# gongweibao/FleetX

Hardware: AMD Instinct MI355X
Metric: tokens/sec (whole node) GPT-3 6.7B hybrid-parallel at 1/2/4/8 MI355X (higher is better)
Workload: dtype bf16; 1 GPU; model=gpt3-6.7B, global_batch=8, seq_len=1024, parallelism=dp1, micro_batch=8, hip_graph=True, grad_reduce_dtype=float32, recompute=False

## Files before the change

### csrc/kernels/norm_eltwise.hip

```cpp
#include "fx_api.h"
#include "fx_common.h"

namespace {

struct DropCfg {
  uint32_t klo, khi, thr;
  float scale;
  int enabled;
  const uint64_t* salt;
};

__device__ __forceinline__ DropCfg resolve_drop(DropCfg d) {
  if (d.enabled && d.salt != nullptr) {
    const uint64_t k = salt_key(((uint64_t)d.khi << 32) | d.klo, *d.salt);
    d.klo = (uint32_t)k;
    d.khi = (uint32_t)(k >> 32);
  }
  return d;
}

__device__ __forceinline__ float drop_apply(float v, uint64_t idx, const DropCfg& d) {
  if (!d.enabled) return v;
  uint32_t h = elem_rand_pair(idx, d.klo, d.khi);
  uint32_t r = (idx & 1) ? (h >> 16) : (h & 0xffffu);
// ... 83 lines not shown
  for (int i = 0; i < VPT; ++i) {
    if (MASK && (i * 64 + lane) * 8 >= h) continue;
#pragma unroll
    for (int j = 0; j < 8; ++j) {
      float d = v[i][j] - mean;
      var += d * d;
    }
  }
  const float rstd = rsqrtf(wave_sum(var) / h + eps);
#pragma unroll
  for (int i = 0; i < VPT; ++i) {
    const int c = (i * 64 + lane) * 8;
    if (MASK && c >= h) continue;
    float g[8], b[8], o[8];
    load8<T>(gamma + c, g);
    load8<T>(beta + c, b);
#pragma unroll
    for (int j = 0; j < 8; ++j) o[j] = (v[i][j] - mean) * rstd * g[j] + b[j];
    store8<T>(y + base + c, o);
  }
  if (lane == 0) {
    mean_out[row] = mean;
    rstd_out[row] = rstd;
  }
}

template <typename T>
__global__ __launch_bounds__(256) void add_ln_fwd_generic(
    const uint16_t* __restrict__ x, const uint16_t* __restrict__ bias,
    const uint16_t* __restrict__ residual, const uint16_t* __restrict__ gamma,
    const uint16_t* __restrict__ beta, uint16_t* __restrict__ s_out,
    uint16_t* __restrict__ y, float* __restrict__ mean_out, float* __restrict__ rstd_out,
    int rows, int h, float eps, DropCfg drop_) {
  const DropCfg drop = resolve_drop(drop_);
  const int lane = threadIdx.x & 63;
  const int row = blockIdx.x * 4 + (threadIdx.x >> 6);
  if (row >= rows) return;
  const size_t base = (size_t)row * h;
  const int nv = h / 8;
  auto value = [&](int c, float* v) {
    load8<T>(x + base + c, v);
    if (bias) {
      float b[8];
      load8<T>(bias + c, b);
      for (int j = 0; j < 8; ++j) v[j] += b[j];
    }
    if (drop.enabled)
      drop_apply8(v, base + c, drop);
    if (residual) {
      float r[8];
      load8<T>(residual + base + c, r);
      for (int j = 0; j < 8; ++j) v[j] += r[j];
    }
  };
  float sum = 0.f;
  for (int vi = lane; vi < nv; vi += 64) {
    float v[8];
    value(vi * 8, v);
    if (s_out) {
      store8<T>(s_out + base + vi * 8, v);
      for (int j = 0; j < 8; ++j) v[j] = round_to<T>(v[j]);
    }
    for (int j = 0; j < 8; ++j) sum += v[j];
  }
  const float mean = wave_sum(sum) / h;
  float var = 0.f;
  for (int vi = lane; vi < nv; vi += 64) {
    float v[8];
    if (s_out) load8<T>(s_out + base + vi * 8, v); else value(vi * 8, v);
    for (int j = 0; j < 8; ++j) { float d = v[j] - mean; var += d * d; }
  }
  const float rstd = rsqrtf(wave_sum(var) / h + eps);
  for (int vi = lane; vi < nv; vi += 64) {
    float v[8], g[8], b[8], o[8];
    if (s_out) load8<T>(s_out + base + vi * 8, v); else value(vi * 8, v);
    load8<T>(gamma + vi * 8, g);
    load8<T>(beta + vi * 8, b);
    for (int j = 0; j < 8; ++j) o[j] = (v[j] - mean) * rstd * g[j] + b[j];
    store8<T>(y + base + vi * 8, o);
  }
  if (lane == 0) { mean_out[row] = mean; rstd_out[row] = rstd; }
}

template <typename T, int VPT, bool MASK = false>
__global__ __launch_bounds__(256) void ln_bwd_row_kernel(
    const uint16_t* __restrict__ dy, const uint16_t* __restrict__ s,
    const float* __restrict__ mean_in, const float* __restrict__ rstd_in,
    const uint16_t* __restrict__ gamma, const uint16_t* __restrict__ ds_in,
    uint16_t* __restrict__ ds_out, uint16_t* __restrict__ dx_out, int rows, int h,
    DropCfg drop_) {
  const DropCfg drop = resolve_drop(drop_);
  const int lane = threadIdx.x & 63;
  const int row = blockIdx.x * 4 + (threadIdx.x >> 6);
  if (row >= rows) return;
  const size_t base = (size_t)row * h;
  const float mean = mean_in[row], rstd = rstd_in[row];
  float xh[VPT][8], gdy[VPT][8];
  float s1 = 0.f, s2 = 0.f;
#pragma unroll
  for (int i = 0; i < VPT; ++i) {
    const int c = (i * 64 + lane) * 8;
    if (MASK && c >= h) {
#pragma unroll
      for (int j = 0; j < 8; ++j) xh[i][j] = gdy[i][j] = 0.f;
      continue;
    }
    float a[8], g[8], d[8];
    load8<T>(s + base + c, a);
    load8<T>(gamma + c, g);
    load8<T>(dy + base + c, d);
#pragma unroll
    for (int j = 0; j < 8; ++j) {
      xh[i][j] = (a[j] - mean) * rstd;
      gdy[i][j] = d[j] * g[j];
      s1 += gdy[i][j];
      s2 += gdy[i][j] * xh[i][j];
    }
  }
  uint4 dr[VPT];
  if (ds_in) {
#pragma unroll
    for (int i = 0; i < VPT; ++i) {
      const int c = (i * 64 + lane) * 8;
      dr[i] = make_uint4(0, 0, 0, 0);
      if (!MASK || c < h) dr[i] = *reinterpret_cast<const uint4*>(ds_in + base + c);
    }
  }
  const float m1 = wave_sum(s1) / h, m2 = wave_sum(s2) / h;
#pragma unroll
  for (int i = 0; i < VPT; ++i) {
    const int c = (i * 64 + lane) * 8;
    if (MASK && c >= h) continue;
    float o[8];
#pragma unroll
    for (int j = 0; j < 8; ++j) o[j] = rstd * (gdy[i][j] - m1 - xh[i][j] * m2);
    if (ds_in) {
      float r[8];
      unpack8<T>(dr[i], r);
#pragma unroll
      for (int j = 0; j < 8; ++j) o[j] += r[j];
    }
    store8<T>(ds_out + base + c, o);
    if (drop.enabled) {
      drop_apply8(o, base + c, drop);
      store8<T>(dx_out + base + c, o);
    } else if (dx_out != ds_out) {
      store8<T>(dx_out + base + c, o);
    }
  }
}

template <typename T>
__global__ __launch_bounds__(256) void ln_bwd_row_generic(
    const uint16_t* __restrict__ dy, const uint16_t* __restrict__ s,
    const float* __restrict__ mean_in, const float* __restrict__ rstd_in,
    const uint16_t* __restrict__ gamma, const uint16_t* __restrict__ ds_in,
    uint16_t* __restrict__ ds_out, uint16_t* __restrict__ dx_out, int rows, int h,
    DropCfg drop_) {
  const DropCfg drop = resolve_drop(drop_);
  const int lane = threadIdx.x & 63;
  const int row = blockIdx.x * 4 + (threadIdx.x >> 6);
  if (row >= rows) return;
  const size_t base = (size_t)row * h;
  const float mean = mean_in[row], rstd = rstd_in[row];
  const int nv = h / 8;
  float s1 = 0.f, s2 = 0.f;
  for (int vi = lane; vi < nv; vi += 64) {
    float a[8], g[8], d[8];
    load8<T>(s + base + vi * 8, a);
    load8<T>(gamma + vi * 8, g);
    load8<T>(dy + base + vi * 8, d);
    for (int j = 0; j < 8; ++j) {
      float xh = (a[j] - mean) * rstd, gd = d[j] * g[j];
      s1 += gd;
      s2 += gd * xh;
    }
  }
  const float m1 = wave_sum(s1) / h, m2 = wave_sum(s2) / h;
  for (int vi = lane; vi < nv; vi += 64) {
    const int c = vi * 8;
    float a[8], g[8], d[8], o[8];
    load8<T>(s + base + c, a);
    load8<T>(gamma + c, g);
    load8<T>(dy + base + c, d);
    for (int j = 0; j < 8; ++j) o[j] = rstd * (d[j] * g[j] - m1 - (a[j] - mean) * rstd * m2);
    if (ds_in) {
      float r[8];
      load8<T>(ds_in + base + c, r);
      for (int j = 0; j < 8; ++j) o[j] += r[j];
    }
    store8<T>(ds_out + base + c, o);
    if (drop.enabled) {
      drop_apply8(o, base + c, drop);
      store8<T>(dx_out + base + c, o);
    } else if (dx_out != ds_out) {
      store8<T>(dx_out + base + c, o);
    }
  }
}

template <typename T, int VPT, int WPR, bool MASK, bool DB>
__global__ __launch_bounds__(256, 2) void ln_bwd_cols_kernel(
    const uint16_t* __restrict__ dy, const uint16_t* __restrict__ s,
    const float* __restrict__ mean_in, const float* __restrict__ rstd_in,
    const uint16_t* __restrict__ gamma, const uint16_t* __restrict__ ds_in,
    uint16_t* __restrict__ ds_out, uint16_t* __restrict__ dx_out, int rows, int h,
    int rows_per_group, float* __restrict__ part, DropCfg drop_) {
  constexpr int NG = 4 / WPR;
  __shared__ float red[4 * 512 * VPT];
  __shared__ float xs[2][4][2];
  const DropCfg drop = resolve_drop(drop_);
  const int lane = threadIdx.x & 63, w = threadIdx.x >> 6;
  const int grp = w / WPR, half = w % WPR;
  const int hw = h / WPR, cbase = half * hw;
  const int r0 = min(rows, (blockIdx.x * NG + grp) * rows_per_group);
  const int r1 = min(rows, r0 + rows_per_group);
  uint4 gp[VPT];
  float ag[VPT][8], ab[VPT][8], ax[DB ? VPT : 1][8];
#pragma unroll
  for (int i = 0; i < VPT; ++i) {
    const int c = (i * 64 + lane) * 8;
    gp[i] = (!MASK || c < hw) ? *reinterpret_cast<const uint4*>(gamma + cbase + c)
                              : make_uint4(0, 0, 0, 0);
#pragma unroll
    for (int j = 0; j < 8; ++j) {
      ag[i][j] = ab[i][j] = 0.f;
      if (DB) ax[i][j] = 0.f;
    }
  }
  for (int k = 0; k < rows_per_group; ++k) {
    const int r = r0 + k;
    const bool live = r < r1;
    if (WPR == 1 && !live) break;
    const size_t base = (size_t)(live ? r : 0) * h + cbase;
    uint4 ca[VPT], cd[VPT], cr[VPT];
    float mean = 0.f, rstd = 0.f, s1 = 0.f, s2 = 0.f;
    if (live) {
#pragma unroll
      for (int i = 0; i < VPT; ++i) {
        const int c = (i * 64 + lane) * 8;
        if (MASK && c >= hw) continue;
        ca[i] = *reinterpret_cast<const uint4*>(s + base + c);
        cd[i] = *reinterpret_cast<const uint4*>(dy + base + c);
      }
      if (ds_in) {
#pragma unroll
        for (int i = 0; i < VPT; ++i) {
          const int c = (i * 64 + lane) * 8;
          if (MASK && c >= hw) continue;
          cr[i] = *reinterpret_cast<const uint4*>(ds_in + base + c);
        }
      }
      mean = mean_in[r];
      rstd = rstd_in[r];
#pragma unroll
      for (int i = 0; i < VPT; ++i) {
        const int c = (i * 64 + lane) * 8;
        if (MASK && c >= hw) continue;
        float a[8], d[8], g[8];
        unpack8<T>(ca[i], a);
        unpack8<T>(cd[i], d);
        unpack8<T>(gp[i], g);
#pragma unroll
        for (int j = 0; j < 8; ++j) {
          const float xh = (a[j] - mean) * rstd, gd = d[j] * g[j];
          s1 += gd;
          s2 += gd * xh;
          ag[i][j] += d[j] * xh;
          ab[i][j] += d[j];
        }
      }
    }
    s1 = wave_sum(s1);
    s2 = wave_sum(s2);
    if constexpr (WPR > 1) {
      if (lane == 0) {
        xs[k & 1][w][0] = s1;
        xs[k & 1][w][1] = s2;
      }
      __syncthreads();
      s1 = xs[k & 1][WPR * grp][0];
      s2 = xs[k & 1][WPR * grp][1];
#pragma unroll
      for (int q = 1; q < WPR; ++q) {
        s1 += xs[k & 1][WPR * grp + q][0];
        s2 += xs[k & 1][WPR * grp + q][1];
      }
    }
    if (!live) continue;
    const float m1 = s1 / h, m2 = s2 / h;
#pragma unroll
    for (int i = 0; i < VPT; ++i) {
      const int c = (i * 64 + lane) * 8;
      if (MASK && c >= hw) continue;
      float a[8], d[8], g[8], o[8];
      unpack8<T>(ca[i], a);
      unpack8<T>(cd[i], d);
      unpack8<T>(gp[i], g);
#pragma unroll
      for (int j = 0; j < 8; ++j) o[j] = rstd * (d[j] * g[j] - m1 - (a[j] - mean) * rstd * m2);
      if (ds_in) {
        float rr[8];
        unpack8<T>(cr[i], rr);
#pragma unroll
        for (int j = 0; j < 8; ++j) o[j] += rr[j];
      }
      store8<T>(ds_out + base + c, o);
      if (drop.enabled) {
        drop_apply8(o, base + c, drop);
        store8<T>(dx_out + base + c, o);
      } else if (dx_out != ds_out) {
        store8<T>(dx_out + base + c, o);
      }
      if (DB) {
#pragma unroll
        for (int j = 0; j < 8; ++j) ax[i][j] += round_to<T>(o[j]);
      }
    }
  }
#pragma unroll
  for (int arr = 0; arr < (DB ? 3 : 2); ++arr) {
    __syncthreads();
#pragma unroll
    for (int i = 0; i < VPT; ++i) {
      const int c = (i * 64 + lane) * 8;
      if (MASK && c >= hw) continue;
#pragma unroll
      for (int j = 0; j < 8; ++j)
        red[grp * h + cbase + c + j] = arr == 0 ? ag[i][j] : arr == 1 ? ab[i][j] : ax[DB ? i : 0][j];
    }
    __syncthreads();
    float* out = part + ((size_t)arr * gridDim.x + blockIdx.x) * h;
    for (int c = threadIdx.x; c < h; c += 256) {
      float v = red[c];
#pragma unroll
      for (int q = 1; q < NG; ++q) v += red[q * h + c];
      out[c] = v;
    }
  }
}

struct LnColsOut {
  float* f32[3];
  uint16_t* t16[3];
  int acc[3];
};
template <typename T>
__global__ __launch_bounds__(256) void ln_cols_finalize_kernel(const float* __restrict__ part,
                                                               int G, int h, LnColsOut f) {
  __shared__ float tr[8][132];
  const int arr = blockIdx.y;
  const float* p = part + (size_t)arr * G * h;
  const int q = threadIdx.x & 31, sr = threadIdx.x >> 5;
  const int c0 = blockIdx.x * 128 + q * 4;
  floatx4 acc = {0.f, 0.f, 0.f, 0.f};
  if (c0 < h) {
    for (int k0 = sr; k0 < G; k0 += 128) {
      floatx4 v[16];
#pragma unroll
      for (int u = 0; u < 16; ++u) {
        const int k = k0 + 8 * u;
        v[u] = k < G ? *reinterpret_cast<const floatx4*>(p + (size_t)k * h + c0)
                     : floatx4{0.f, 0.f, 0.f, 0.f};
      }
#pragma unroll
      for (int u = 0; u < 16; ++u) acc += v[u];
    }
  }
#pragma unroll
  for (int j = 0; j < 4; ++j) tr[sr][q * 4 + j] = acc[j];
  __syncthreads();
  const int c = threadIdx.x, gc = blockIdx.x * 128 + c;
  if (c >= 128 || gc >= h) return;
  float sum = 0.f;
#pragma unroll
  for (int t = 0; t < 8; ++t) sum += tr[t][c];
  if (f.f32[arr]) f.f32[arr][gc] = f.acc[arr] ? f.f32[arr][gc] + sum : sum;
  if (f.t16[arr]) f.t16[arr][gc] = Elt<T>::from_f(sum);
}

typedef __attribute__((address_space(1))) float gf32;
typedef __attribute__((address_space(1))) int gi32;

__device__ __forceinline__ void st_part(float* p, float v) {
  __hip_atomic_store((gf32*)p, v, __ATOMIC_RELAXED, __HIP_MEMORY_SCOPE_AGENT);
}

struct ColFin {
  int* cnt;
  float* f32[2];
  uint16_t* t16[2];
  int acc[2];
};

template <typename T>
__device__ __forceinline__ void colsum_tail(const float* __restrict__ p0,
                                            const float* __restrict__ p1, int cols, int np,
                                            const ColFin& f) {
  __shared__ int last;
  asm volatile("s_waitcnt vmcnt(0)" ::: "memory");
  __syncthreads();
  if (threadIdx.x == 0) {
    const int t = __hip_atomic_fetch_add((gi32*)(f.cnt + 32 * blockIdx.x), 1, __ATOMIC_RELAXED,
                                         __HIP_MEMORY_SCOPE_AGENT);
    last = t == (int)gridDim.y - 1;
    if (last)
      __hip_atomic_store((gi32*)(f.cnt + 32 * blockIdx.x), 0, __ATOMIC_RELAXED,
                         __HIP_MEMORY_SCOPE_AGENT);
  }
  __syncthreads();
  if (!last) return;
  __builtin_amdgcn_fence(__ATOMIC_ACQUIRE, "wavefront");
  __shared__ float tr[8][132];
  const int q = threadIdx.x & 31, sr = threadIdx.x >> 5;
  const int c0 = blockIdx.x * 128 + q * 4;
  const int splits = gridDim.y;
  for (int which = 0; which < np; ++which) {
    const float* p = which ? p1 : p0;
    floatx4 s = {0.f, 0.f, 0.f, 0.f};
    if (c0 < cols) {
      const auto rs = __builtin_amdgcn_make_buffer_rsrc(const_cast<float*>(p), 0,
                                                        splits * cols * 4, 0x00020000);
      for (int k0 = sr; k0 < splits; k0 += 128) {
        floatx4 v[16];
#pragma unroll
        for (int u = 0; u < 16; ++u) {
          const int k = k0 + 8 * u;
          const uint32_t off = k < splits ? (uint32_t)(k * cols + c0) * 4u : 0x80000000u;
          v[u] = __builtin_bit_cast(floatx4, __builtin_amdgcn_raw_buffer_load_b128(rs, off, 0, 16));
        }
#pragma unroll
        for (int u = 0; u < 16; ++u) s += v[u];
      }
    }
#pragma unroll
    for (int j = 0; j < 4; ++j) tr[sr][q * 4 + j] = s[j];
    __syncthreads();
    const int c = threadIdx.x, gc = blockIdx.x * 128 + c;
    if (c < 128 && gc < cols) {
      float sum = 0.f;
#pragma unroll
      for (int t = 0; t < 8; ++t) sum += tr[t][c];
      if (f.f32[which]) f.f32[which][gc] = f.acc[which] ? f.f32[which][gc] + sum : sum;
      if (f.t16[which]) f.t16[which][gc] = Elt<T>::from_f(sum);
    }
    __syncthreads();
  }
}

template <typename T, int MODE>
__global__ __launch_bounds__(256) void coltile_partial_kernel(
    const uint16_t* __restrict__ a, const uint16_t* __restrict__ b,
    const float* __restrict__ mean, const float* __restrict__ rstd,
    float* __restrict__ p0, float* __restrict__ p1, int rows, int cols, int rows_per_split,
    ColFin fin) {
  __shared__ float red[2][16][129];
  const int tx = threadIdx.x & 15, ty = threadIdx.x >> 4;
  const int col = blockIdx.x * 128 + tx * 8;
  const int r0 = blockIdx.y * rows_per_split;
// ... 318 lines not shown
  DropCfg d = make_drop(p, key, salt);
  dim3 grid((rows + 3) / 4), block(256);
  auto X = (const uint16_t*)x;
  auto B = (const uint16_t*)bias;
  auto R = (const uint16_t*)residual;
  auto G = (const uint16_t*)gamma;
  auto Be = (const uint16_t*)beta;
  auto S = (uint16_t*)s_out;
  auto Y = (uint16_t*)y;
#define LN_CASE(V)                                                                          \
  case V:                                                                                   \
    FX_DISPATCH_T(dtype, add_ln_fwd_kernel<T, V><<<grid, block, 0, st>>>(                   \
                             X, B, R, G, Be, S, Y, mean, rstd, rows, h, eps, d));           \
    break;
  if (h % 512 == 0 && h / 512 <= 16) {
    switch (h / 512) {
      LN_CASE(1) LN_CASE(2) LN_CASE(3) LN_CASE(4) LN_CASE(5) LN_CASE(6) LN_CASE(7) LN_CASE(8)
      LN_CASE(10) LN_CASE(12) LN_CASE(16)
      default:
        FX_DISPATCH_T(dtype, add_ln_fwd_generic<T><<<grid, block, 0, st>>>(
                                 X, B, R, G, Be, S, Y, mean, rstd, rows, h, eps, d));
    }
  } else if (h % 8 == 0 && h < 8 * 512) {
#define LNM_CASE(V)                                                                          \
  case V:                                                                                    \
    FX_DISPATCH_T(dtype, add_ln_fwd_kernel<T, V, true><<<grid, block, 0, st>>>(              \
                             X, B, R, G, Be, S, Y, mean, rstd, rows, h, eps, d));            \
    break;
    switch ((h + 511) / 512) {
      LNM_CASE(1) LNM_CASE(2) LNM_CASE(3) LNM_CASE(4) LNM_CASE(5) LNM_CASE(6) LNM_CASE(7)
      LNM_CASE(8)
    }
#undef LNM_CASE
  } else {
    FX_DISPATCH_T(dtype, add_ln_fwd_generic<T><<<grid, block, 0, st>>>(
                             X, B, R, G, Be, S, Y, mean, rstd, rows, h, eps, d));
  }
#undef LN_CASE
}

extern "C" void fx_ln_bwd_row(int dtype, const void* dy, const void* s, const float* mean,
                              const float* rstd, const void* gamma, const void* ds_in,
                              void* ds_out, void* dx_out, int rows, int h, float p, uint64_t key,
                              const void* salt, hipStream_t st) {
  DropCfg d = make_drop(p, key, salt);
  dim3 grid((rows + 3) / 4), block(256);
  auto DY = (const uint16_t*)dy;
  auto S = (const uint16_t*)s;
  auto G = (const uint16_t*)gamma;
  auto DI = (const uint16_t*)ds_in;
  auto DS = (uint16_t*)ds_out;
  auto DX = (uint16_t*)dx_out;
#define LNB_CASE(V)                                                                       \
  case V:                                                                                 \
    FX_DISPATCH_T(dtype, ln_bwd_row_kernel<T, V><<<grid, block, 0, st>>>(                 \
                             DY, S, mean, rstd, G, DI, DS, DX, rows, h, d));              \
    break;
  if (h % 512 == 0 && h / 512 <= 8) {
    switch (h / 512) {
      LNB_CASE(1) LNB_CASE(2) LNB_CASE(3) LNB_CASE(4) LNB_CASE(5) LNB_CASE(6) LNB_CASE(7)
      LNB_CASE(8)
      default:
        FX_DISPATCH_T(dtype, ln_bwd_row_generic<T><<<grid, block, 0, st>>>(
                                 DY, S, mean, rstd, G, DI, DS, DX, rows, h, d));
    }
  } else if (h % 8 == 0 && h < 8 * 512) {
#define LNBM_CASE(V)                                                                      \
  case V:                                                                                 \
    FX_DISPATCH_T(dtype, ln_bwd_row_kernel<T, V, true><<<grid, block, 0, st>>>(           \
                             DY, S, mean, rstd, G, DI, DS, DX, rows, h, d));              \
    break;
    switch ((h + 511) / 512) {
      LNBM_CASE(1) LNBM_CASE(2) LNBM_CASE(3) LNBM_CASE(4) LNBM_CASE(5) LNBM_CASE(6)
      LNBM_CASE(7) LNBM_CASE(8)
    }
#undef LNBM_CASE
  } else {
    FX_DISPATCH_T(dtype, ln_bwd_row_generic<T><<<grid, block, 0, st>>>(
                             DY, S, mean, rstd, G, DI, DS, DX, rows, h, d));
  }
#undef LNB_CASE
}

static int ln_cols_wpr(int h) { return h <= 1536 ? 1 : h <= 3072 ? 2 : 4; }
static int ln_cols_rows_per_group(int rows, int h) {
  const int ng = 4 / ln_cols_wpr(h);
  int rpg = (rows + 512 * ng - 1) / (512 * ng);
  return rpg < 2 ? 2 : rpg;
}
extern "C" int fx_ln_bwd_cols_blocks(int rows, int h, int max_h) {
  if (rows <= 0 || h > (max_h < 4096 ? max_h : 4096) || h % (8 * ln_cols_wpr(h))) return 0;
  const int ng = 4 / ln_cols_wpr(h), rpg = ln_cols_rows_per_group(rows, h);
  return (rows + ng * rpg - 1) / (ng * rpg);
}

extern "C" int fx_ln_bwd_cols(int dtype, const void* dy, const void* s, const float* mean,
                              const float* rstd, const void* gamma, const void* ds_in,
                              void* ds_out, void* dx_out, int rows, int h, float p, uint64_t key,
                              float* part, int with_dbias, float* fg, void* tg, int accg,
                              float* fb, void* tb, int accb, float* fx, void* tx, int accx,
                              const void* salt, hipStream_t st) {
  const int G = fx_ln_bwd_cols_blocks(rows, h, 4096);
  if (G == 0) return -1;
  const int wpr = ln_cols_wpr(h), hw = h / wpr;
  const int rpg = ln_cols_rows_per_group(rows, h);
  DropCfg d = make_drop(p, key, salt);
  auto DY = (const uint16_t*)dy;
  auto S = (const uint16_t*)s;
  auto GM = (const uint16_t*)gamma;
  auto DI = (const uint16_t*)ds_in;
  auto DS = (uint16_t*)ds_out;
  auto DX = (uint16_t*)dx_out;
  const int vpt = (hw + 511) / 512;
  const bool mask = hw % 512 != 0;
#define LNC_GO(V, W, M, DB)                                                                   \
  FX_DISPATCH_T(dtype, ln_bwd_cols_kernel<T, V, W, M, DB><<<G, 256, 0, st>>>(                 \
                           DY, S, mean, rstd, GM, DI, DS, DX, rows, h, rpg, part, d))
#define LNC_M(V, W)                                                                           \
  if (mask) {                                                                                 \
    if (with_dbias) { LNC_GO(V, W, true, true); } else { LNC_GO(V, W, true, false); }         \
  } else {                                                                                    \
    if (with_dbias) { LNC_GO(V, W, false, true); } else { LNC_GO(V, W, false, false); }       \
  }
#define LNC_V(V)                                                                              \
  case V:                                                                                     \
    if (wpr == 1) { LNC_M(V, 1) } else if (wpr == 2) { LNC_M(V, 2) } else { LNC_M(V, 4) }     \
    break;
  switch (vpt) {
    LNC_V(1) LNC_V(2) LNC_V(3)
    default: return -1;
  }
#undef LNC_V
#undef LNC_M
#undef LNC_GO
  LnColsOut f;
  f.f32[0] = fg; f.f32[1] = fb; f.f32[2] = fx;
  f.t16[0] = (uint16_t*)tg; f.t16[1] = (uint16_t*)tb; f.t16[2] = (uint16_t*)tx;
  f.acc[0] = accg; f.acc[1] = accb; f.acc[2] = accx;
  dim3 grid((h + 127) / 128, with_dbias ? 3 : 2);
  FX_DISPATCH_T(dtype, ln_cols_finalize_kernel<T><<<grid, 256, 0, st>>>(part, G, h, f));
  return 0;
}

extern "C" void fx_coltile_partial(int dtype, int mode, const void* a, const void* b,
                                   const float* mean, const float* rstd, float* p0, float* p1,
                                   int rows, int cols, int splits, hipStream_t st, int* cnt,
                                   float* f0, void* t0, int acc0, float* f1, void* t1, int acc1) {
  const ColFin fin = make_fin(cnt, f0, t0, acc0, f1, t1, acc1);
  int rps = (rows + splits - 1) / splits;
  dim3 grid((cols + 127) / 128, splits), block(256);
  auto A = (const uint16_t*)a;
  auto B = (const uint16_t*)b;
  if (mode == 0) {
    FX_DISPATCH_T(dtype, coltile_partial_kernel<T, 0><<<grid, block, 0, st>>>(
                             A, B, mean, rstd, p0, p1, rows, cols, rps, fin));
  } else {
    FX_DISPATCH_T(dtype, coltile_partial_kernel<T, 1><<<grid, block, 0, st>>>(
                             A, B, mean, rstd, p0, p1, rows, cols, rps, fin));
  }
}

extern "C" void fx_coltile_finalize(int dtype, const float* part, int splits, int cols,
                                    float* out_f32, void* out_t, int accumulate, hipStream_t st) {
  dim3 grid((cols + 255) / 256), block(256);
  FX_DISPATCH_T(dtype, coltile_finalize_kernel<T><<<grid, block, 0, st>>>(
                           part, splits, cols, out_f32, (uint16_t*)out_t, accumulate));
}

extern "C" void fx_bias_gelu_fwd(int dtype, int erf, const void* x, const void* bias, void* y,
                                 long n, int cols, hipStream_t st) {
  long n8 = n / 8;
  if (erf) {
    FX_DISPATCH_T(dtype, bias_gelu_fwd_kernel<T, true><<<grid_for(n8), 256, 0, st>>>(
                             (const uint16_t*)x, (const uint16_t*)bias, (uint16_t*)y, n8, cols));
  } else {
    FX_DISPATCH_T(dtype, bias_gelu_fwd_kernel<T, false><<<grid_for(n8), 256, 0, st>>>(
                             (const uint16_t*)x, (const uint16_t*)bias, (uint16_t*)y, n8, cols));
  }
}

extern "C" void fx_bias_gelu_bwd(int dtype, int erf, const void* dy, const void* x,
                                 const void* bias, void* dx, float* part, int rows, int cols,
                                 int splits, hipStream_t st, int* cnt, float* out_f32,
                                 void* out_t, int acc) {
  const ColFin fin = make_fin(cnt, out_f32, out_t, acc, nullptr, nullptr, 0);
  int rps = (rows + splits - 1) / splits;
  dim3 grid((cols + 127) / 128, splits), block(256);
  if (erf) {
    FX_DISPATCH_T(dtype, bias_gelu_bwd_kernel<T, true><<<grid, block, 0, st>>>(
                             (const uint16_t*)dy, (const uint16_t*)x, (const uint16_t*)bias,
                             (uint16_t*)dx, part, rows, cols, rps, fin));
  } else {
    FX_DISPATCH_T(dtype, bias_gelu_bwd_kernel<T, false><<<grid, block, 0, st>>>(
                             (const uint16_t*)dy, (const uint16_t*)x, (const uint16_t*)bias,
                             (uint16_t*)dx, part, rows, cols, rps, fin));
  }
}

extern "C" void fx_bias_dropout_add_fwd(int dtype, const void* x, const void* bias,
                                        const void* residual, void* out, long n, int cols, float p,
                                        uint64_t key, const void* salt, hipStream_t st) {
  DropCfg d = make_drop(p, key, salt);
  long n8 = n / 8;
  FX_DISPATCH_T(dtype, bias_dropout_add_fwd_kernel<T><<<grid_for(n8), 256, 0, st>>>(
                           (const uint16_t*)x, (const uint16_t*)bias, (const uint16_t*)residual,
                           (uint16_t*)out, n8, cols, d));
}

extern "C" void fx_dropout_bwd_colsum(int dtype, const void* dout, void* dx, float* part,
                                      int rows, int cols, int splits, float p, uint64_t key,
                                      const void* salt, hipStream_t st, int* cnt,
                                      float* out_f32, void* out_t, int acc) {
  const ColFin fin = make_fin(cnt, out_f32, out_t, acc, nullptr, nullptr, 0);
  DropCfg d = make_drop(p, key, salt);
  int rps = (rows + splits - 1) / splits;
  dim3 grid((cols + 127) / 128, splits), block(256);
  FX_DISPATCH_T(dtype, dropout_bwd_colsum_kernel<T><<<grid, block, 0, st>>>(
                           (const uint16_t*)dout, (uint16_t*)dx, part, rows, cols, rps, d, fin));
}

extern "C" void fx_dropout_fwd(int dtype, const void* x, void* y, long n, float p, uint64_t key,
                               const void* salt, hipStream_t st) {
  DropCfg d = make_drop(p, key, salt);
// ... 5 lines not shown
```

### fleetx_amd/ops/norm.py

```python
import os

import torch

from . import _lib
from ..parallel import grad_sink as sink, rng as _rng


_TICKETS = {}


def colsum_tickets(device, cols):
    st = torch.cuda.current_stream(device).cuda_stream
    need = 32 * ((cols + 127) // 128)
    t = _TICKETS.get(st)
    if t is None or t.numel() < need:
        t = torch.zeros(max(4096, need), dtype=torch.int32, device=device)
        _TICKETS[st] = t
    return t.data_ptr()


_TARGET_KW = (("f0", "t0", "acc0"), ("f1", "t1", "acc1"))


def _coltile(mode, x, aux, rows, cols, targets):
    k = _lib.kernels()
    splits = k.coltile_splits(rows, cols)
    p0 = torch.empty(splits, cols, device=x.device, dtype=torch.float32)
    p1 = torch.empty_like(p0) if mode == 0 else None
    fin = {}
    for (kf, kt, ka), (f32, t16, acc) in zip(_TARGET_KW, targets):
        if f32:
            fin[kf], fin[ka] = f32, acc
        else:
            fin[kt] = t16
    k.coltile_partial(_lib.dt_code(x.dtype), mode, x.data_ptr(), *aux, p0.data_ptr(),
                      _lib.ptr(p1), rows, cols, splits, _lib.stream(),
                      cnt=colsum_tickets(x.device, cols), **fin)


def _col_target(prm, direct, cols, like):
    if direct:
        mg, acc = sink.open_write(prm)
        return (mg.data_ptr(), 0, int(acc)), None
    g = torch.empty(cols, device=like.device, dtype=like.dtype)
    return (0, g.data_ptr(), 0), g


def col_sum(x, cols):
    if not _lib.vec8_ok(cols, x):
        return x.reshape(-1, cols).float().sum(0).to(x.dtype)
    out = torch.empty(cols, device=x.device, dtype=x.dtype)
    _coltile(1, x, (0, 0, 0), x.numel() // cols, cols, [(0, out.data_ptr(), 0)])
    return out


def col_sum_f32(x, dst, accumulate=False):
    cols = dst.numel()
    x = x.contiguous()
    if not _lib.vec8_ok(cols, x):
        sink.store_or_add(dst, x.reshape(-1, cols).float().sum(0).view_as(dst), accumulate)
        return dst
    if dst.dtype != torch.float32 or not dst.is_contiguous():
        raise ValueError("col_sum_f32: dst must be contiguous fp32")
    _coltile(1, x, (0, 0, 0), x.numel() // cols, cols, [(dst.data_ptr(), 0, int(accumulate))])
    return dst


def _dropout_ref(x, p, key):
    if p <= 0.0:
        return x
    m = _rng.keep_mask(x.shape, p, key, x.device)
    return torch.where(m, x * (1.0 / (1.0 - p)), torch.zeros_like(x))


def _ln_bwd_cols_max_h():
    mode = os.environ.get("FLEETX_LN_BWD_FUSED", "1")
    return {"0": 0, "2": 4096}.get(mode, 1536)


def _ln_bwd_cols(k, dc, dy, s, mean, rstd, weight, ctx, ds_in, ds, dx, rows, h):
    G = k.ln_bwd_cols_blocks(rows, h, 4096)
    with_db = bool(ctx.has_bias)
    part = torch.empty(3 if with_db else 2, G, h, device=dy.device, dtype=torch.float32)
    prms = (weight, ctx.lnbias, ctx.bias if with_db else None)
    outs, grads = [], []
    for prm in prms:
        t, g = ((0, 0, 0), None) if prm is None else \
            _col_target(prm, sink.fused(prm, fp32_contiguous=True), h, dy)
        outs.append(t)
        grads.append(g)
    (fg, tg, ag), (fb, tb, ab), (fx, tx, ax) = outs
    rc = k.ln_bwd_cols(dc, dy.data_ptr(), s.data_ptr(), mean.data_ptr(), rstd.data_ptr(),
                       weight.data_ptr(), _lib.ptr(ds_in), ds.data_ptr(), dx.data_ptr(), rows, h,
                       float(ctx.p), ctx.key, part.data_ptr(), int(with_db), fg, tg, ag, fb, tb,
                       ab, fx, tx, ax, _rng.device_salt_ptr(), _lib.stream())
    if rc != 0:
        raise RuntimeError("ln_bwd_cols: shape rows=%d h=%d not covered" % (rows, h))
    for prm, (f32, _, _) in zip(prms, outs):
        if f32:
            sink.close_write(prm)
    return grads


class _AddLayerNorm(torch.autograd.Function):
    @staticmethod
    def forward(ctx, x, bias, residual, weight, lnbias, eps, p, key, store_sum):
        h = x.shape[-1]
        rows = x.numel() // h
        ctx.p, ctx.key, ctx.has_bias, ctx.has_res = p, key, bias is not None, residual is not None
        ctx.h = h
        x = x.contiguous()
        if _lib.vec8_ok(h, x, bias, residual, weight, lnbias):
            k = _lib.kernels()
            fused = bias is not None or residual is not None or p > 0
            s = torch.empty_like(x) if fused else None
            y = torch.empty_like(x)
            mean = torch.empty(rows, device=x.device, dtype=torch.float32)
            rstd = torch.empty_like(mean)
            k.add_ln_fwd(_lib.dt_code(x.dtype), x.data_ptr(), _lib.ptr(bias), _lib.ptr(residual),
                         weight.data_ptr(), lnbias.data_ptr(), _lib.ptr(s), y.data_ptr(),
                         mean.data_ptr(), rstd.data_ptr(), rows, h, float(eps), float(p), key,
                         _rng.device_salt_ptr(), _lib.stream())
            s_saved = s if s is not None else x
            if s is None and store_sum:
                s = x
        else:
            v = x
            if bias is not None or residual is not None or p > 0:
                v = x.float() if bias is None else x.float() + bias.float()
                v = _dropout_ref(v, p, key)
                if residual is not None:
                    v = v + residual.float()
                v = v.to(x.dtype)
            s_saved = v
            s = v if (store_sum or bias is not None or residual is not None or p > 0) else None
            vf = v.float()
            mean = vf.mean(-1).reshape(-1)
            var = ((vf - mean.view(*vf.shape[:-1], 1)) ** 2).mean(-1).reshape(-1)
            rstd = torch.rsqrt(var + eps)
            y = ((vf - mean.view(*vf.shape[:-1], 1)) * rstd.view(*vf.shape[:-1], 1) * weight.float()
                 + lnbias.float()).to(x.dtype)
        ctx.save_for_backward(s_saved, mean, rstd, weight)
        ctx.lnbias, ctx.bias = lnbias, bias
        ctx.return_sum = s is not None
        if s is None:
            return y
        return s, y

    @staticmethod
    def backward(ctx, *grads):
        if ctx.return_sum:
            ds_in, dy = grads
        else:
            ds_in, dy = None, grads[0]
        s, mean, rstd, weight = ctx.saved_tensors
        h = ctx.h
        rows = s.numel() // h
        dy = dy.contiguous()
        if ds_in is not None:
            ds_in = ds_in.contiguous()
# ... 76 lines not shown
```

Measured before the change: 28580 tokens/s.

## Add wide fused LayerNorm backward with column reductions and enable it by default

Adds a new ln_bwd_wide_kernel for hidden sizes above 1536 (GPT-3 6.7B uses 4096). It computes dx together with the per-column gamma, beta and bias gradient partials in one pass, using prefetch of the next row and LDS-resident accumulators. A double-precision wide finalize kernel reduces the partials. The multi-wave-per-row path is removed, and the default FLEETX_LN_BWD_FUSED max h goes from 1536 to 4096, so h=4096 now takes the fused path instead of a separate row kernel plus column sums. This trades extra LDS and register pressure and a partial buffer for fewer passes over activations.

```diff
diff --git a/csrc/kernels/norm_eltwise.hip b/csrc/kernels/norm_eltwise.hip
--- a/csrc/kernels/norm_eltwise.hip
+++ b/csrc/kernels/norm_eltwise.hip
@@ -189,6 +189,47 @@
   if (lane == 0) { mean_out[row] = mean; rstd_out[row] = rstd; }
 }
 
+__device__ __forceinline__ void ln_bwd_stats8(const float* a, const float* d, const float* g,
+                                              float mean, float rstd, float* xh, float& s1,
+                                              float& s2) {
+#pragma clang fp contract(off)
+#pragma unroll
+  for (int j = 0; j < 8; ++j) {
+    xh[j] = (a[j] - mean) * rstd;
+    const float gd = d[j] * g[j];
+    const float gx = gd * xh[j];
+    s1 = s1 + gd;
+    s2 = s2 + gx;
+  }
+}
+template <typename T>
+__device__ __forceinline__ void ln_bwd_out8(const float* d, const float* g, const float* xh,
+                                            float m1, float m2, float rstd, bool has_in,
+                                            const uint4& in, float* o) {
+#pragma clang fp contract(off)
+#pragma unroll
+  for (int j = 0; j < 8; ++j)
+    o[j] = rstd * __builtin_fmaf(-m2, xh[j], __builtin_fmaf(d[j], g[j], -m1));
+  if (has_in) {
+    float r[8];
+    unpack8<T>(in, r);
+#pragma unroll
+    for (int j = 0; j < 8; ++j) o[j] = o[j] + r[j];
+  }
+}
+template <typename T>
+__device__ __forceinline__ uint4 pack8_exact(const float* f) {
+  uint4 v;
+  uint16_t* h = reinterpret_cast<uint16_t*>(&v);
+#pragma unroll
+  for (int j = 0; j < 8; ++j) {
+    float q = f[j];
+    asm volatile("" : "+v"(q));
+    h[j] = Elt<T>::from_f(q);
+  }
+  return v;
+}
+
 template <typename T, int VPT, bool MASK = false>
 __global__ __launch_bounds__(256) void ln_bwd_row_kernel(
     const uint16_t* __restrict__ dy, const uint16_t* __restrict__ s,
@@ -202,27 +243,21 @@
   if (row >= rows) return;
   const size_t base = (size_t)row * h;
   const float mean = mean_in[row], rstd = rstd_in[row];
-  float xh[VPT][8], gdy[VPT][8];
+  float xh[VPT][8], g[VPT][8], d[VPT][8];
   float s1 = 0.f, s2 = 0.f;
 #pragma unroll
   for (int i = 0; i < VPT; ++i) {
     const int c = (i * 64 + lane) * 8;
     if (MASK && c >= h) {
 #pragma unroll
-      for (int j = 0; j < 8; ++j) xh[i][j] = gdy[i][j] = 0.f;
+      for (int j = 0; j < 8; ++j) xh[i][j] = g[i][j] = d[i][j] = 0.f;
       continue;
     }
-    float a[8], g[8], d[8];
+    float a[8];
     load8<T>(s + base + c, a);
-    load8<T>(gamma + c, g);
-    load8<T>(dy + base + c, d);
-#pragma unroll
-    for (int j = 0; j < 8; ++j) {
-      xh[i][j] = (a[j] - mean) * rstd;
-      gdy[i][j] = d[j] * g[j];
-      s1 += gdy[i][j];
-      s2 += gdy[i][j] * xh[i][j];
-    }
+    load8<T>(gamma + c, g[i]);
+    load8<T>(dy + base + c, d[i]);
+    ln_bwd_stats8(a, d[i], g[i], mean, rstd, xh[i], s1, s2);
   }
   uint4 dr[VPT];
   if (ds_in) {
@@ -239,20 +274,14 @@
     const int c = (i * 64 + lane) * 8;
     if (MASK && c >= h) continue;
     float o[8];
-#pragma unroll
-    for (int j = 0; j < 8; ++j) o[j] = rstd * (gdy[i][j] - m1 - xh[i][j] * m2);
-    if (ds_in) {
-      float r[8];
-      unpack8<T>(dr[i], r);
-#pragma unroll
-      for (int j = 0; j < 8; ++j) o[j] += r[j];
-    }
-    store8<T>(ds_out + base + c, o);
+    ln_bwd_out8<T>(d[i], g[i], xh[i], m1, m2, rstd, ds_in != nullptr, dr[i], o);
+    const uint4 pk = pack8_exact<T>(o);
+    *reinterpret_cast<uint4*>(ds_out + base + c) = pk;
     if (drop.enabled) {
       drop_apply8(o, base + c, drop);
-      store8<T>(dx_out + base + c, o);
+      *reinterpret_cast<uint4*>(dx_out + base + c) = pack8_exact<T>(o);
     } else if (dx_out != ds_out) {
-      store8<T>(dx_out + base + c, o);
+      *reinterpret_cast<uint4*>(dx_out + base + c) = pk;
     }
   }
 }
@@ -306,20 +335,18 @@
   }
 }
 
-template <typename T, int VPT, int WPR, bool MASK, bool DB>
+template <typename T, int VPT, bool MASK, bool DB>
 __global__ __launch_bounds__(256, 2) void ln_bwd_cols_kernel(
     const uint16_t* __restrict__ dy, const uint16_t* __restrict__ s,
     const float* __restrict__ mean_in, const float* __restrict__ rstd_in,
     const uint16_t* __restrict__ gamma, const uint16_t* __restrict__ ds_in,
     uint16_t* __restrict__ ds_out, uint16_t* __restrict__ dx_out, int rows, int h,
     int rows_per_group, float* __restrict__ part, DropCfg drop_) {
-  constexpr int NG = 4 / WPR;
+  constexpr int NG = 4;
   __shared__ float red[4 * 512 * VPT];
-  __shared__ float xs[2][4][2];
   const DropCfg drop = resolve_drop(drop_);
-  const int lane = threadIdx.x & 63, w = threadIdx.x >> 6;
-  const int grp = w / WPR, half = w % WPR;
-  const int hw = h / WPR, cbase = half * hw;
+  const int lane = threadIdx.x & 63, grp = threadIdx.x >> 6;
+  const int hw = h, cbase = 0;
   const int r0 = min(rows, (blockIdx.x * NG + grp) * rows_per_group);
   const int r1 = min(rows, r0 + rows_per_group);
   uint4 gp[VPT];
@@ -337,12 +364,11 @@
   }
   for (int k = 0; k < rows_per_group; ++k) {
     const int r = r0 + k;
-    const bool live = r < r1;
-    if (WPR == 1 && !live) break;
-    const size_t base = (size_t)(live ? r : 0) * h + cbase;
+    if (r >= r1) break;
+    const size_t base = (size_t)r * h + cbase;
     uint4 ca[VPT], cd[VPT], cr[VPT];
     float mean = 0.f, rstd = 0.f, s1 = 0.f, s2 = 0.f;
-    if (live) {
+    {
 #pragma unroll
       for (int i = 0; i < VPT; ++i) {
         const int c = (i * 64 + lane) * 8;
@@ -380,21 +406,6 @@
     }
     s1 = wave_sum(s1);
     s2 = wave_sum(s2);
-    if constexpr (WPR > 1) {
-      if (lane == 0) {
-        xs[k & 1][w][0] = s1;
-        xs[k & 1][w][1] = s2;
-      }
-      __syncthreads();
-      s1 = xs[k & 1][WPR * grp][0];
-      s2 = xs[k & 1][WPR * grp][1];
-#pragma unroll
-      for (int q = 1; q < WPR; ++q) {
-        s1 += xs[k & 1][WPR * grp + q][0];
-        s2 += xs[k & 1][WPR * grp + q][1];
-      }
-    }
-    if (!live) continue;
     const float m1 = s1 / h, m2 = s2 / h;
 #pragma unroll
     for (int i = 0; i < VPT; ++i) {
@@ -445,6 +456,186 @@
       out[c] = v;
     }
   }
+}
+
+template <typename T, int VPT, bool MASK, bool DB>
+__global__ __launch_bounds__(256) void ln_bwd_wide_kernel(
+    const uint16_t* __restrict__ dy, const uint16_t* __restrict__ s,
+    const float* __restrict__ mean_in, const float* __restrict__ rstd_in,
+    const uint16_t* __restrict__ gamma, const uint16_t* __restrict__ ds_in,
+    uint16_t* __restrict__ ds_out, uint16_t* __restrict__ dx_out, int rows, int h,
+    int rows_per_wave, int wave_rows, float* __restrict__ part, DropCfg drop_) {
+  constexpr int WR = 512 * VPT;
+  __shared__ floatx4 acc_lds[(DB ? 2 : 1) * 4 * WR / 4];
+  const DropCfg drop = resolve_drop(drop_);
+  const int lane = threadIdx.x & 63;
+  const int w = __builtin_amdgcn_readfirstlane(threadIdx.x >> 6);
+  const int r0 = min(rows, (blockIdx.x * 4 + w) * rows_per_wave);
+  const int r1 = min(rows, r0 + rows_per_wave);
+  floatx4* const lb = acc_lds + w * (WR / 4) + lane;
+  floatx4* const lx = lb + (DB ? 4 * (WR / 4) : 0);
+  __shared__ uint4 gam_lds[64 * VPT];
+  for (int v = threadIdx.x; v < 64 * VPT; v += 256)
+    gam_lds[v] = (!MASK || v * 8 < h) ? *reinterpret_cast<const uint4*>(gamma + v * 8)
+                                      : make_uint4(0, 0, 0, 0);
+  float ag[VPT][8];
+#pragma unroll
+  for (int i = 0; i < VPT; ++i) {
+#pragma unroll
+    for (int j = 0; j < 8; ++j) ag[i][j] = 0.f;
+#pragma unroll
+    for (int q = 0; q < 2; ++q) {
+      lb[(2 * i + q) * 64] = floatx4{0.f, 0.f, 0.f, 0.f};
+      if (DB) lx[(2 * i + q) * 64] = floatx4{0.f, 0.f, 0.f, 0.f};
+    }
+  }
+  uint4 ca[VPT], cd[VPT], cr[VPT];
+  float mean_n = 0.f, rstd_n = 0.f;
+  if (r0 < r1) {
+    const size_t base = (size_t)r0 * h;
+#pragma unroll
+    for (int i = 0; i < VPT; ++i) {
+      const int c = (i * 64 + lane) * 8;
+      ca[i] = cd[i] = cr[i] = make_uint4(0, 0, 0, 0);
+      if (MASK && c >= h) continue;
+      ca[i] = *reinterpret_cast<const uint4*>(s + base + c);
+      cd[i] = *reinterpret_cast<const uint4*>(dy + base + c);
+    }
+    if (ds_in) {
+#pragma unroll
+      for (int i = 0; i < VPT; ++i) {
+        const int c = (i * 64 + lane) * 8;
+        if (MASK && c >= h) continue;
+        cr[i] = *reinterpret_cast<const uint4*>(ds_in + base + c);
+      }
+    }
+    mean_n = mean_in[r0];
+    rstd_n = rstd_in[r0];
+  }
+  __syncthreads();
+  for (int r = r0; r < r1; ++r) {
+    const size_t base = (size_t)r * h;
+    const float mean = mean_n, rstd = rstd_n;
+    float xh[VPT][8];
+    uint4 dk[VPT];
+    float s1 = 0.f, s2 = 0.f;
+#pragma unroll
+    for (int i = 0; i < VPT; ++i) {
+      const int c = (i * 64 + lane) * 8;
+      dk[i] = cd[i];
+      if (MASK && c >= h) {
+#pragma unroll
+        for (int j = 0; j < 8; ++j) xh[i][j] = 0.f;
+        continue;
+      }
+      float a[8], g[8], d[8];
+      unpack8<T>(ca[i], a);
+      unpack8<T>(gam_lds[i * 64 + lane], g);
+      unpack8<T>(cd[i], d);
+      ln_bwd_stats8(a, d, g, mean, rstd, xh[i], s1, s2);
+      floatx4 b0 = lb[(2 * i) * 64], b1 = lb[(2 * i + 1) * 64];
+#pragma unroll
+      for (int j = 0; j < 8; ++j) ag[i][j] += d[j] * xh[i][j];
+#pragma unroll
+      for (int e = 0; e < 4; ++e) {
+        b0[e] += d[e];
+        b1[e] += d[4 + e];
+      }
+      lb[(2 * i) * 64] = b0;
+      lb[(2 * i + 1) * 64] = b1;
+    }
+    const bool more = r + 1 < r1;
+    if (more) {
+      const size_t nb = base + h;
+#pragma unroll
+      for (int i = 0; i < VPT; ++i) {
+        const int c = (i * 64 + lane) * 8;
+        if (MASK && c >= h) continue;
+        ca[i] = *reinterpret_cast<const uint4*>(s + nb + c);
+        cd[i] = *reinterpret_cast<const uint4*>(dy + nb + c);
+      }
+      mean_n = mean_in[r + 1];
+      rstd_n = rstd_in[r + 1];
+    }
+    const float m1 = wave_sum(s1) / h, m2 = wave_sum(s2) / h;
+#pragma unroll
+    for (int i = 0; i < VPT; ++i) {
+      const int c = (i * 64 + lane) * 8;
+      if (MASK && c >= h) continue;
+      float g[8], d[8], o[8];
+      unpack8<T>(gam_lds[i * 64 + lane], g);
+      unpack8<T>(dk[i], d);
+      ln_bwd_out8<T>(d, g, xh[i], m1, m2, rstd, ds_in != nullptr, cr[i], o);
+      uint4 pk = pack8_exact<T>(o);
+      *reinterpret_cast<uint4*>(ds_out + base + c) = pk;
+      if (drop.enabled) {
+        drop_apply8(o, base + c, drop);
+        pk = pack8_exact<T>(o);
+        *reinterpret_cast<uint4*>(dx_out + base + c) = pk;
+      } else if (dx_out != ds_out) {
+        *reinterpret_cast<uint4*>(dx_out + base + c) = pk;
+      }
+      if (DB) {
+        float xf[8];
+        unpack8<T>(pk, xf);
+        floatx4 x0 = lx[(2 * i) * 64], x1 = lx[(2 * i + 1) * 64];
+#pragma unroll
+        for (int e = 0; e < 4; ++e) {
+          x0[e] += xf[e];
+          x1[e] += xf[4 + e];
+        }
+        lx[(2 * i) * 64] = x0;
+        lx[(2 * i + 1) * 64] = x1;
+      }
+    }
+    if (more && ds_in) {
+      const size_t nb = base + h;
+#pragma unroll
+      for (int i = 0; i < VPT; ++i) {
+        const int c = (i * 64 + lane) * 8;
+        if (MASK && c >= h) continue;
+        cr[i] = *reinterpret_cast<const uint4*>(ds_in + nb + c);
+      }
+    }
+  }
+  if (wave_rows) {
+    const size_t G = (size_t)gridDim.x * 4, row = (size_t)blockIdx.x * 4 + w;
+#pragma unroll
+    for (int i = 0; i < VPT; ++i) {
+      const int c = (i * 64 + lane) * 8;
+      if (MASK && c >= h) continue;
+#pragma unroll
+      for (int q = 0; q < 2; ++q) {
+        *reinterpret_cast<floatx4*>(part + row * h + c + 4 * q) =
+            floatx4{ag[i][4 * q], ag[i][4 * q + 1], ag[i][4 * q + 2], ag[i][4 * q + 3]};
+        *reinterpret_cast<floatx4*>(part + (G + row) * h + c + 4 * q) = lb[(2 * i + q) * 64];
+        if (DB) *reinterpret_cast<floatx4*>(part + (2 * G + row) * h + c + 4 * q) = lx[(2 * i + q) * 64];
+      }
+    }
+    return;
+  }
+  const float* const red = reinterpret_cast<const float*>(acc_lds);
+  auto block_sum = [&](int arr, int region) {
+    float* out = part + ((size_t)arr * gridDim.x + blockIdx.x) * h;
+    for (int c = threadIdx.x; c < h; c += 256) {
+      const int off = region * 4 * WR + (((c >> 9) * 2 + ((c >> 2) & 1)) * 64 + ((c >> 3) & 63)) * 4 + (c & 3);
+      double v = red[off];
+#pragma unroll
+      for (int q = 1; q < 4; ++q) v += (double)red[q * WR + off];
+      out[c] = (float)v;
+    }
+  };
+  __syncthreads();
+  block_sum(1, 0);
+  if (DB) block_sum(2, 1);
+  __syncthreads();
+#pragma unroll
+  for (int i = 0; i < VPT; ++i) {
+    lb[(2 * i) * 64] = floatx4{ag[i][0], ag[i][1], ag[i][2], ag[i][3]};
+    lb[(2 * i + 1) * 64] = floatx4{ag[i][4], ag[i][5], ag[i][6], ag[i][7]};
+  }
+  __syncthreads();
+  block_sum(0, 0);
 }
 
 struct LnColsOut {
@@ -482,6 +673,42 @@
   float sum = 0.f;
 #pragma unroll
   for (int t = 0; t < 8; ++t) sum += tr[t][c];
+  if (f.f32[arr]) f.f32[arr][gc] = f.acc[arr] ? f.f32[arr][gc] + sum : sum;
+  if (f.t16[arr]) f.t16[arr][gc] = Elt<T>::from_f(sum);
+}
+
+template <typename T>
+__global__ __launch_bounds__(256) void ln_cols_finalize_wide_kernel(
+    const float* __restrict__ part, int G, int h, LnColsOut f) {
+  __shared__ double tr[32][33];
+  typedef double doublex4 __attribute__((ext_vector_type(4)));
+  const int arr = blockIdx.y;
+  const float* p = part + (size_t)arr * G * h;
+  const int q = threadIdx.x & 7, sr = threadIdx.x >> 3;
+  const int c0 = blockIdx.x * 32 + q * 4;
+  doublex4 acc = {0., 0., 0., 0.};
+  if (c0 < h) {
+    for (int k0 = sr; k0 < G; k0 += 512) {
+      floatx4 v[16];
+#pragma unroll
+      for (int u = 0; u < 16; ++u) {
+        const int k = k0 + 32 * u;
+        v[u] = k < G ? *reinterpret_cast<const floatx4*>(p + (size_t)k * h + c0)
+                     : floatx4{0.f, 0.f, 0.f, 0.f};
+      }
+#pragma unroll
+      for (int u = 0; u < 16; ++u) acc += __builtin_convertvector(v[u], doublex4);
+    }
+  }
+#pragma unroll
+  for (int j = 0; j < 4; ++j) tr[sr][q * 4 + j] = acc[j];
+  __syncthreads();
+  const int c = threadIdx.x, gc = blockIdx.x * 32 + c;
+  if (c >= 32 || gc >= h) return;
+  double sumd = 0.;
+#pragma unroll
+  for (int t = 0; t < 32; ++t) sumd += tr[t][c];
+  const float sum = (float)sumd;
   if (f.f32[arr]) f.f32[arr][gc] = f.acc[arr] ? f.f32[arr][gc] + sum : sum;
   if (f.t16[arr]) f.t16[arr][gc] = Elt<T>::from_f(sum);
 }
@@ -966,16 +1193,18 @@
 #undef LNB_CASE
 }
 
-static int ln_cols_wpr(int h) { return h <= 1536 ? 1 : h <= 3072 ? 2 : 4; }
 static int ln_cols_rows_per_group(int rows, int h) {
-  const int ng = 4 / ln_cols_wpr(h);
-  int rpg = (rows + 512 * ng - 1) / (512 * ng);
-  return rpg < 2 ? 2 : rpg;
-}
+  const int rpg = (rows + 512 * 4 - 1) / (512 * 4);
+  return h <= 1536 && rpg < 2 ? 2 : rpg;
+}
+static int ln_cols_grid(int rows, int h) {
+  const int rpg = ln_cols_rows_per_group(rows, h);
+  return (rows + 4 * rpg - 1) / (4 * rpg);
+}
+static bool ln_cols_wave_rows(int rows, int h) { return h > 1536 && 4 * ln_cols_grid(rows, h) <= 512; }
 extern "C" int fx_ln_bwd_cols_blocks(int rows, int h, int max_h) {
-  if (rows <= 0 || h > (max_h < 4096 ? max_h : 4096) || h % (8 * ln_cols_wpr(h))) return 0;
-  const int ng = 4 / ln_cols_wpr(h), rpg = ln_cols_rows_per_group(rows, h);
-  return (rows + ng * rpg - 1) / (ng * rpg);
+  if (rows <= 0 || h > (max_h < 4096 ? max_h : 4096) || h % 8) return 0;
+  return ln_cols_grid(rows, h) * (ln_cols_wave_rows(rows, h) ? 4 : 1);
 }
 
 extern "C" int fx_ln_bwd_cols(int dtype, const void* dy, const void* s, const float* mean,
@@ -986,8 +1215,7 @@
                               const void* salt, hipStream_t st) {
   const int G = fx_ln_bwd_cols_blocks(rows, h, 4096);
   if (G == 0) return -1;
-  const int wpr = ln_cols_wpr(h), hw = h / wpr;
-  const int rpg = ln_cols_rows_per_group(rows, h);
+  const int rpg = ln_cols_rows_per_group(rows, h), nblk = ln_cols_grid(rows, h);
   DropCfg d = make_drop(p, key, salt);
   auto DY = (const uint16_t*)dy;
   auto S = (const uint16_t*)s;
@@ -995,34 +1223,43 @@
   auto DI = (const uint16_t*)ds_in;
   auto DS = (uint16_t*)ds_out;
   auto DX = (uint16_t*)dx_out;
-  const int vpt = (hw + 511) / 512;
-  const bool mask = hw % 512 != 0;
-#define LNC_GO(V, W, M, DB)                                                                   \
-  FX_DISPATCH_T(dtype, ln_bwd_cols_kernel<T, V, W, M, DB><<<G, 256, 0, st>>>(                 \
-                           DY, S, mean, rstd, GM, DI, DS, DX, rows, h, rpg, part, d))
-#define LNC_M(V, W)                                                                           \
-  if (mask) {                                                                                 \
-    if (with_dbias) { LNC_GO(V, W, true, true); } else { LNC_GO(V, W, true, false); }         \
-  } else {                                                                                    \
-    if (with_dbias) { LNC_GO(V, W, false, true); } else { LNC_GO(V, W, false, false); }       \
-  }
-#define LNC_V(V)                                                                              \
+  const int vpt = (h + 511) / 512;
+  const bool mask = h % 512 != 0;
+#define LNC_GO(K, V, M, DB)                                                                   \
+  FX_DISPATCH_T(dtype, K<T, V, M, DB><<<nblk, 256, 0, st>>>(DY, S, mean, rstd, GM, DI, DS, DX,    \
+                                                            rows, h, rpg, LNC_EXTRA part, d))
+#define LNC_V(K, V)                                                                           \
   case V:                                                                                     \
-    if (wpr == 1) { LNC_M(V, 1) } else if (wpr == 2) { LNC_M(V, 2) } else { LNC_M(V, 4) }     \
+    if (mask) {                                                                               \
+      if (with_dbias) { LNC_GO(K, V, true, true); } else { LNC_GO(K, V, true, false); }       \
+    } else {                                                                                  \
+      if (with_dbias) { LNC_GO(K, V, false, true); } else { LNC_GO(K, V, false, false); }     \
+    }                                                                                         \
     break;
+  const int wave_rows = ln_cols_wave_rows(rows, h);
   switch (vpt) {
-    LNC_V(1) LNC_V(2) LNC_V(3)
+#define LNC_EXTRA
+    LNC_V(ln_bwd_cols_kernel, 1) LNC_V(ln_bwd_cols_kernel, 2) LNC_V(ln_bwd_cols_kernel, 3)
+#undef LNC_EXTRA
+#define LNC_EXTRA wave_rows,
+    LNC_V(ln_bwd_wide_kernel, 4) LNC_V(ln_bwd_wide_kernel, 5) LNC_V(ln_bwd_wide_kernel, 6)
+    LNC_V(ln_bwd_wide_kernel, 7) LNC_V(ln_bwd_wide_kernel, 8)
+#undef LNC_EXTRA
     default: return -1;
   }
 #undef LNC_V
-#undef LNC_M
 #undef LNC_GO
   LnColsOut f;
   f.f32[0] = fg; f.f32[1] = fb; f.f32[2] = fx;
   f.t16[0] = (uint16_t*)tg; f.t16[1] = (uint16_t*)tb; f.t16[2] = (uint16_t*)tx;
   f.acc[0] = accg; f.acc[1] = accb; f.acc[2] = accx;
-  dim3 grid((h + 127) / 128, with_dbias ? 3 : 2);
-  FX_DISPATCH_T(dtype, ln_cols_finalize_kernel<T><<<grid, 256, 0, st>>>(part, G, h, f));
+  if (vpt <= 3) {
+    dim3 grid((h + 127) / 128, with_dbias ? 3 : 2);
+    FX_DISPATCH_T(dtype, ln_cols_finalize_kernel<T><<<grid, 256, 0, st>>>(part, G, h, f));
+  } else {
+    dim3 grid((h + 31) / 32, with_dbias ? 3 : 2);
+    FX_DISPATCH_T(dtype, ln_cols_finalize_wide_kernel<T><<<grid, 256, 0, st>>>(part, G, h, f));
+  }
   return 0;
 }
 
diff --git a/fleetx_amd/ops/norm.py b/fleetx_amd/ops/norm.py
--- a/fleetx_amd/ops/norm.py
+++ b/fleetx_amd/ops/norm.py
@@ -74,8 +74,8 @@
 
 
 def _ln_bwd_cols_max_h():
-    mode = os.environ.get("FLEETX_LN_BWD_FUSED", "1")
-    return {"0": 0, "2": 4096}.get(mode, 1536)
+    mode = os.environ.get("FLEETX_LN_BWD_FUSED", "2")
+    return {"0": 0, "1": 1536}.get(mode, 4096)
 
 
 def _ln_bwd_cols(k, dc, dy, s, mean, rstd, weight, ctx, ds_in, ds, dx, rows, h):
```

Result: no change. 28620 tokens/s (median of 3 runs) (+0.1%).
